# SobeyMIL/MVOC

Measured on AMD Instinct MI355X. Metric: UNet3D denoising steps/sec, 16x512^2 frames, inversion+compose, higher is better.
Workload: dtype f16

## Files before the change

mvoc_amd/csrc/attention.hip:

```cpp
#include <stdlib.h>

#include "common.h"

namespace {

typedef __fp16 fp16x4_t __attribute__((__vector_size__(4 * sizeof(__fp16))));
template <int D> struct FlashPitch { static constexpr int K = 2 * D + 16, V = D == 64 ? 192 : 320; };

struct AttnArgs {
  const half_t *q, *k, *v;
  half_t* out;
  long q_bs, q_ts, k_bs, k_ts, v_bs, v_ts, o_bs, o_ts;
  int nbatch, heads, tq, tk, kv_bdiv, causal;
  float scale_log2;
  long v2_off, o2_off;
  int qblocks;
};

__device__ __forceinline__ int vt_slot_group(int key) {
  return ((((key >> 5) * 2 + ((key >> 4) & 1)) * 2) + ((key >> 2) & 1));
}
__device__ __forceinline__ int vt_slot_elem(int key) { return ((key >> 3) & 1) * 4 + (key & 3); }

constexpr float FLASH_THR = 8.0f;

typedef float f32x2 __attribute__((ext_vector_type(2)));
__device__ __forceinline__ float flash_xhalf_max(float x) {
  const unsigned u = __builtin_bit_cast(unsigned, x);
  const auto sw = __builtin_amdgcn_permlane32_swap(u, u, false, false);
  return fmaxf(__builtin_bit_cast(float, (unsigned)sw[0]), __builtin_bit_cast(float, (unsigned)sw[1]));
}

template <int D, int NV>
#ifndef FLASH_MINW
#define FLASH_MINW 4
#endif
__global__ __launch_bounds__(256, (D == 64 && NV == 1) ? FLASH_MINW : 1) void flash_kernel(const AttnArgs p) {
  constexpr int KPITCH = FlashPitch<D>::K, VPITCH = FlashPitch<D>::V;
  constexpr int ND = D / 16, NT = D / 32, CPK = D / 8, NCH = 64 * CPK / 256;
  __shared__ __attribute__((aligned(16))) char smem[64 * KPITCH + NV * 64 * VPITCH];
  char* Ks = smem;
  char* Vs = smem + 64 * KPITCH;
  const int tid = threadIdx.x, lane = tid & 63;
  const int wave = __builtin_amdgcn_readfirstlane(tid >> 6);
  const int r = lane & 31, h = lane >> 5;
  const unsigned logical = xcd_remap(blockIdx.x, gridDim.x);
  const unsigned qb_ = logical % (unsigned)p.qblocks, hb_ = logical / (unsigned)p.qblocks;
  const int head = (int)(hb_ % (unsigned)p.heads), b = (int)(hb_ / (unsigned)p.heads);
  const int q0 = (int)qb_ * 128 + wave * 32;

  const half_t* qp = p.q + (long)b * p.q_bs + head * D;
  const int qrow = min(q0 + r, p.tq - 1);
  half8_t qf[ND];
#pragma unroll
  for (int s = 0; s < ND; ++s) qf[s] = *reinterpret_cast<const half8_t*>(qp + (long)qrow * p.q_ts + 16 * s + 8 * h);

  const char* kb = reinterpret_cast<const char*>(p.k + (long)(b / p.kv_bdiv) * p.k_bs + head * D);
  const char* vb = reinterpret_cast<const char*>(p.v + (long)(b / p.kv_bdiv) * p.v_bs + head * D);
  const unsigned k_rb = (unsigned)p.k_ts * 2u, v_rb = (unsigned)p.v_ts * 2u;
  unsigned koff[NCH], voff[NCH];
#pragma unroll
  for (int i = 0; i < NCH; ++i) {
    const int c = tid + i * 256;
    koff[i] = (unsigned)(c / CPK) * k_rb + (unsigned)(c % CPK) * 16u;
    voff[i] = (unsigned)(c / CPK) * v_rb + (unsigned)(c % CPK) * 16u;
  }

  f32x16 ot[NV][NT];
#pragma unroll
  for (int v = 0; v < NV; ++v)
#pragma unroll
    for (int dt = 0; dt < NT; ++dt)
#pragma unroll
      for (int e = 0; e < 16; ++e) ot[v][dt][e] = 0.f;
  float mrun = -INFINITY, lrun = 0.f;

  const int ntiles = (p.tk + 63) / 64;
  half8_t kreg[NCH], vreg[NV][NCH];
  auto gload = [&](int kt) {
    const char* kt_ = kb + (size_t)kt * 64u * k_rb;
    const char* vt_ = vb + (size_t)kt * 64u * v_rb;
    const bool ragged = __builtin_amdgcn_readfirstlane(kt * 64 + 64 > p.tk);
#pragma unroll
    for (int i = 0; i < NCH; ++i) {
      unsigned ko = koff[i], vo = voff[i];
      if (ragged) {
        const int c = tid + i * 256;
        const unsigned row = (unsigned)min(c / CPK, p.tk - 1 - kt * 64);
        ko = row * k_rb + (unsigned)(c % CPK) * 16u;
        vo = row * v_rb + (unsigned)(c % CPK) * 16u;
      }
      kreg[i] = *reinterpret_cast<const half8_t*>(kt_ + ko);
#pragma unroll
      for (int v = 0; v < NV; ++v) vreg[v][i] = *reinterpret_cast<const half8_t*>(vt_ + (size_t)v * (size_t)p.v2_off * 2u + vo);
    }
  };
  gload(0);
  for (int kt = 0; kt < ntiles; ++kt) {
    __syncthreads();
#pragma unroll
    for (int i = 0; i < NCH; ++i) {
      const int c = tid + i * 256;
      const int key = c / CPK, dc = c % CPK;
      *reinterpret_cast<half8_t*>(Ks + key * KPITCH + dc * 16) = kreg[i];
#pragma unroll
      for (int v = 0; v < NV; ++v)
        *reinterpret_cast<half8_t*>(Vs + v * 64 * VPITCH + key * VPITCH + dc * 16) = vreg[v][i];
    }
    __syncthreads();
    if (kt + 1 < ntiles) gload(kt + 1);

    f32x16 st[2];
#pragma unroll
    for (int t = 0; t < 2; ++t) {
#pragma unroll
      for (int e = 0; e < 16; ++e) st[t][e] = 0.f;
#pragma unroll
      for (int s = 0; s < ND; ++s) {
        const half8_t kf = *reinterpret_cast<const half8_t*>(Ks + (32 * t + r) * KPITCH + (16 * s + 8 * h) * 2);
        st[t] = __builtin_amdgcn_mfma_f32_32x32x16_f16(kf, qf[s], st[t], 0, 0, 0);
      }
    }
    if (__builtin_amdgcn_readfirstlane((kt == ntiles - 1) && (p.tk & 63))) {
#pragma unroll
      for (int t = 0; t < 2; ++t)
#pragma unroll
        for (int e = 0; e < 16; ++e)
          if (kt * 64 + 32 * t + 8 * (e >> 2) + 4 * h + (e & 3) >= p.tk) st[t][e] = -INFINITY;
    }
    if (p.causal) {
#pragma unroll
      for (int t = 0; t < 2; ++t)
#pragma unroll
        for (int e = 0; e < 16; ++e)
          if (kt * 64 + 32 * t + 8 * (e >> 2) + 4 * h + (e & 3) > q0 + r) st[t][e] = -INFINITY;
    }
    float mx = st[0][0];
#pragma unroll
    for (int t = 0; t < 2; ++t)
#pragma unroll
      for (int e = 0; e < 16; ++e) mx = fmaxf(mx, st[t][e]);
    mx = flash_xhalf_max(mx);
    if (__any((mx - mrun) * p.scale_log2 > FLASH_THR)) {
      const float mnew = fmaxf(mrun, mx);
      const float alpha = __builtin_amdgcn_exp2f((mrun - mnew) * p.scale_log2);
      mrun = mnew;
      lrun *= alpha;
#pragma unroll
      for (int v = 0; v < NV; ++v)
#pragma unroll
        for (int dt = 0; dt < NT; ++dt)
#pragma unroll
          for (int e = 0; e < 16; ++e) ot[v][dt][e] *= alpha;
    }
    const f32x2 sc2 = {p.scale_log2, p.scale_log2}, mc2 = {-mrun * p.scale_log2, -mrun * p.scale_log2};
#pragma unroll
    for (int t = 0; t < 2; ++t)
#pragma unroll
      for (int e = 0; e < 16; e += 2) {
        const f32x2 a = __builtin_elementwise_fma(f32x2{st[t][e], st[t][e + 1]}, sc2, mc2);
        st[t][e] = __builtin_amdgcn_exp2f(a[0]);
        st[t][e + 1] = __builtin_amdgcn_exp2f(a[1]);
      }

#pragma unroll
    for (int t = 0; t < 2; ++t)
#pragma unroll
      for (int s = 0; s < 2; ++s) {
        half8_t pf;
#pragma unroll
        for (int j = 0; j < 8; ++j) pf[j] = (half_t)st[t][8 * s + j];
#pragma unroll
        for (int j = 0; j < 4; ++j) lrun = __builtin_amdgcn_fdot2(half2_t{pf[2 * j], pf[2 * j + 1]}, half2_t{(half_t)1.f, (half_t)1.f}, lrun, false);
        const int krow = 32 * t + 16 * s + 4 * h + ((lane & 15) >> 2);
#pragma unroll
        for (int v = 0; v < NV; ++v)
#pragma unroll
          for (int dt = 0; dt < NT; ++dt) {
            const char* va = Vs + v * 64 * VPITCH + krow * VPITCH + (32 * dt + 16 * ((lane >> 4) & 1) + 4 * (lane & 3)) * 2;
            const fp16x4_t lo = __builtin_amdgcn_ds_read_tr16_b64_v4f16((__attribute__((address_space(3))) fp16x4_t*)va);
            const fp16x4_t hi = __builtin_amdgcn_ds_read_tr16_b64_v4f16((__attribute__((address_space(3))) fp16x4_t*)(va + 8 * VPITCH));
            half8_t vf;
#pragma unroll
            for (int e = 0; e < 4; ++e) {
              vf[e] = (half_t)lo[e];
              vf[4 + e] = (half_t)hi[e];
            }
            ot[v][dt] = __builtin_amdgcn_mfma_f32_32x32x16_f16(vf, pf, ot[v][dt], 0, 0, 0);
          }
      }
  }
  const float ltot = lrun + __shfl_xor(lrun, 32);
  const float inv = 1.0f / ltot;
  int lane_e = tid;
  asm volatile("" : "+v"(lane_e));
  const int r_e = lane_e & 31, h_e = (lane_e >> 5) & 1;
  if (q0 + r_e < p.tq) {
#pragma unroll
    for (int v = 0; v < NV; ++v) {
      half_t* op = p.out + v * p.o2_off + (long)b * p.o_bs + (long)(q0 + r_e) * p.o_ts + head * D;
#pragma unroll
      for (int dt = 0; dt < NT; ++dt)
#pragma unroll
        for (int q = 0; q < 4; ++q) {
          half4_t o;
#pragma unroll
          for (int e = 0; e < 4; ++e) o[e] = (half_t)(ot[v][dt][q * 4 + e] * inv);
          *reinterpret_cast<half4_t*>(op + 32 * dt + 8 * q + 4 * h_e) = o;
        }
    }
  }
}

#define F3_BAR()                         \
  do {                                   \
    __builtin_amdgcn_sched_barrier(0);   \
    __builtin_amdgcn_s_barrier();        \
    __builtin_amdgcn_sched_barrier(0);   \
  } while (0)
#define F3_FENCE() __builtin_amdgcn_sched_barrier(0)
#define F3_GRP(V, T)                                   \
  do {                                                 \
    __builtin_amdgcn_sched_group_barrier(0x008, 1, 0); \
    __builtin_amdgcn_sched_group_barrier(0x002, V, 0); \
    __builtin_amdgcn_sched_group_barrier(0x400, T, 0); \
  } while (0)
#define F3_RD(R) __builtin_amdgcn_sched_group_barrier(0x100, R, 0)
#ifdef MVOC_F3_STAMPS
__device__ unsigned long long f3_dbg[8];
#define F3_STAMP(i)                                                                      \
  do {                                                                                   \
    unsigned long long t_;                                                               \
    asm volatile("s_memtime %0\n\ts_waitcnt lgkmcnt(0)" : "=s"(t_)::"memory");          \
    if (blockIdx.x == 0 && tid == 0) { f3_acc[i] += t_ - f3_last; }                      \
    f3_last = t_;                                                                        \
  } while (0)
#else
#define F3_STAMP(i)
#endif
typedef unsigned u32x4 __attribute__((ext_vector_type(4)));
__device__ __forceinline__ void f3_dma(const u32x4 rsrc, unsigned voff, unsigned lds) {
  unsigned keep;
  asm volatile("s_mov_b32 %0, m0\n\ts_mov_b32 m0, %2\n\ts_nop 0\n\tbuffer_load_dwordx4 %1, %3, 0 offen lds\n\ts_mov_b32 m0, %0"
               : "=&s"(keep) : "v"(voff), "s"(lds), "s"(rsrc) : "memory");
}
__device__ __forceinline__ u32x4 f3_rsrc(const void* base, unsigned bytes) {
  const unsigned long long a = (unsigned long long)base;
  u32x4 r;
  r[0] = __builtin_amdgcn_readfirstlane((unsigned)a);
  r[1] = __builtin_amdgcn_readfirstlane((unsigned)(a >> 32));
  r[2] = __builtin_amdgcn_readfirstlane(bytes);
  r[3] = 0x00020000u;
  return r;
}
template <int N>
__device__ __forceinline__ void f3_wait_vm() {
  asm volatile("s_waitcnt vmcnt(%0)" ::"n"(N) : "memory");
}
#ifndef F3_W1
#define F3_W1 3
#endif
template <int NV>
__global__ __launch_bounds__(256, NV == 1 ? F3_W1 : 2) void flash3_kernel(const AttnArgs p) {
  constexpr int D = 64, NS = (NV == 1 && F3_W1 == 2) ? 4 : 3, TILE = 8192 * (1 + NV), PCS = 2 + 2 * NV;
  __shared__ __attribute__((aligned(1024))) char smem[NS * TILE];
#ifdef MVOC_F3_STAMPS
  unsigned long long f3_acc[6] = {0, 0, 0, 0, 0, 0}, f3_last = 0, f3_t0, f3_r0;
#endif
  const int tid = threadIdx.x, lane = tid & 63;
  const int wave = __builtin_amdgcn_readfirstlane(tid >> 6);
  const int r = lane & 31, h = lane >> 5;
#ifdef MVOC_F3_STAMPS
  asm volatile("s_memtime %0\n\ts_memrealtime %1\n\ts_waitcnt lgkmcnt(0)" : "=s"(f3_t0), "=s"(f3_r0)::"memory");
  f3_last = f3_t0;
#endif
  const unsigned logical = xcd_remap(blockIdx.x, gridDim.x);
  const unsigned qb_ = logical % (unsigned)p.qblocks, hb_ = logical / (unsigned)p.qblocks;
  const int head = (int)(hb_ % (unsigned)p.heads), b = (int)(hb_ / (unsigned)p.heads);
  const int q0 = (int)qb_ * 128 + wave * 32;
  const int nt = (p.tk + 63) >> 6;

  const unsigned k_rb = (unsigned)p.k_ts * 2u, v_rb = (unsigned)p.v_ts * 2u;
  const half_t* kb = p.k + (long)(b / p.kv_bdiv) * p.k_bs + head * D;
  const half_t* vb = p.v + (long)(b / p.kv_bdiv) * p.v_bs + head * D;
  const u32x4 rs_k = f3_rsrc(kb, (unsigned)(p.tk - 1) * k_rb + 128u);
  const u32x4 rs_v0 = f3_rsrc(vb, (unsigned)(p.tk - 1) * v_rb + 128u);
  const u32x4 rs_v1 = f3_rsrc(vb + p.v2_off, (unsigned)(p.tk - 1) * v_rb + 128u);
  unsigned ksrc[2], vsrc[2];
#pragma unroll
  for (int j = 0; j < 2; ++j) {
    const int key_l = 16 * wave + 8 * j + (lane >> 3), pc = lane & 7;
    ksrc[j] = (unsigned)key_l * k_rb + (unsigned)((pc ^ ((key_l >> 1) & 7)) * 16);
    vsrc[j] = (unsigned)key_l * v_rb + (unsigned)((pc ^ (((key_l >> 1) & 1) << 2)) * 16);
  }
  const unsigned ktile = 64u * k_rb, vtile = 64u * v_rb;
  const unsigned lds0 = (unsigned)(size_t)(__attribute__((address_space(3))) char*)smem;
  auto issue = [&](int tile, int so) {
    const unsigned base = lds0 + (unsigned)so + (unsigned)wave * 2048u;
#pragma unroll
    for (int j = 0; j < 2; ++j) f3_dma(rs_k, ksrc[j] + (unsigned)tile * ktile, base + j * 1024);
#pragma unroll
    for (int v = 0; v < NV; ++v)
#pragma unroll
      for (int j = 0; j < 2; ++j) f3_dma(v ? rs_v1 : rs_v0, vsrc[j] + (unsigned)tile * vtile, base + 8192 * (1 + v) + j * 1024);
  };
  const half_t* qp = p.q + (long)b * p.q_bs + head * D;
  const int qrow = min(q0 + r, p.tq - 1);
  half8_t qf[4];
#pragma unroll
  for (int s = 0; s < 4; ++s) qf[s] = *reinterpret_cast<const half8_t*>(qp + (long)qrow * p.q_ts + 16 * s + 8 * h);
  asm volatile("s_nop 4" ::: "memory");
  F3_FENCE();
#pragma unroll
  for (int t = 0; t < NS - 1; ++t) issue(t, t * TILE);
  F3_FENCE();

  f32x16 ot[NV][2];
#pragma unroll
  for (int v = 0; v < NV; ++v)
#pragma unroll
    for (int dt = 0; dt < 2; ++dt)
#pragma unroll
      for (int e = 0; e < 16; ++e) ot[v][dt][e] = 0.f;
  float mrun = -INFINITY, lrun = 0.f;
  f32x16 sa[2], sb[2];
  f32x16 zero16;
#pragma unroll
  for (int e = 0; e < 16; ++e) zero16[e] = 0.f;

  int kfo[4];
#pragma unroll
  for (int s = 0; s < 4; ++s) kfo[s] = r * 128 + (((2 * s + h) ^ ((r >> 1) & 7)) * 16);
  const int vq = (lane & 15) >> 2;
  int vfo[2];
#pragma unroll
  for (int dt = 0; dt < 2; ++dt) vfo[dt] = 8192 + (4 * h + vq) * 128 + (((32 * ((lane >> 4) & 1) + 8 * (lane & 3))) | ((dt ^ ((vq >> 1) & 1)) << 6));

  f3_wait_vm<(NS - 2) * PCS>();
  F3_BAR();
#pragma unroll
  for (int t = 0; t < 2; ++t) {
    sa[t] = zero16;
#pragma unroll
    for (int s = 0; s < 4; ++s) {
      const half8_t kf = *reinterpret_cast<const half8_t*>(smem + kfo[s] + 4096 * t);
      sa[t] = __builtin_amdgcn_mfma_f32_32x32x16_f16(kf, qf[s], sa[t], 0, 0, 0);
    }
  }
  int o_v = 0, o_k = TILE, o_w = (NS - 1) * TILE;

  auto body = [&](f32x16(&cur)[2], f32x16(&nxt)[2], const int t) {
    F3_STAMP(4);
    f3_wait_vm<(NS - 3) * PCS>();
    F3_BAR();
    F3_STAMP(0);
    issue(t + NS - 1, o_w);
    F3_FENCE();
    F3_STAMP(1);
    const char* Kn = smem + o_k;
    const char* Vc = smem + o_v;
    if (__builtin_amdgcn_readfirstlane((t == nt - 1) && (p.tk & 63))) {
#pragma unroll
      for (int tt = 0; tt < 2; ++tt)
#pragma unroll
        for (int e = 0; e < 16; ++e)
          if (t * 64 + 32 * tt + 8 * (e >> 2) + 4 * h + (e & 3) >= p.tk) cur[tt][e] = -INFINITY;
    }
    F3_FENCE();
    half8_t kf[2][4];
#pragma unroll
    for (int s = 0; s < 2; ++s)
#pragma unroll
      for (int tt = 0; tt < 2; ++tt) kf[tt][s] = *reinterpret_cast<const half8_t*>(Kn + kfo[s] + 4096 * tt);
    half8_t pf[2];
    half8_t vf[3][NV][2];
    auto vread = [&](const int f) {
#pragma unroll
      for (int v = 0; v < NV; ++v)
#pragma unroll
        for (int dt = 0; dt < 2; ++dt) {
          const char* va = Vc + 8192 * v + vfo[dt] + (32 * (f >> 1) + 16 * (f & 1)) * 128;
          const fp16x4_t lo = __builtin_amdgcn_ds_read_tr16_b64_v4f16((__attribute__((address_space(3))) fp16x4_t*)va);
          const fp16x4_t hi = __builtin_amdgcn_ds_read_tr16_b64_v4f16((__attribute__((address_space(3))) fp16x4_t*)(va + 8 * 128));
#pragma unroll
          for (int e = 0; e < 4; ++e) {
            vf[f % 3][v][dt][e] = (half_t)lo[e];
            vf[f % 3][v][dt][4 + e] = (half_t)hi[e];
          }
        }
    };
    vread(0);
    F3_FENCE();
    auto smma = [&](const int i) {
      const int tt = i & 1, s_ = i >> 1;
      nxt[tt] = __builtin_amdgcn_mfma_f32_32x32x16_f16(kf[tt][s_], qf[s_], s_ == 0 ? zero16 : nxt[tt], 0, 0, 0);
    };
    auto pvmma = [&](const int f, const int dt) {
#pragma unroll
      for (int v = 0; v < NV; ++v) ot[v][dt] = __builtin_amdgcn_mfma_f32_32x32x16_f16(vf[f % 3][v][dt], pf[f & 1], ot[v][dt], 0, 0, 0);
    };
    float mx = fmaxf(cur[0][0], cur[0][1]);
#pragma unroll
    for (int tt = 0; tt < 2; ++tt)
#pragma unroll
      for (int e = tt ? 0 : 2; e < 16; e += 2) mx = __builtin_fmaxf(__builtin_fmaxf(mx, cur[tt][e]), cur[tt][e + 1]);
    smma(0); smma(1); smma(2);
    if constexpr (NV == 2) smma(3);
    mx = flash_xhalf_max(mx);
    if constexpr (NV == 1) { F3_GRP(6, 0); F3_GRP(6, 0); F3_GRP(6, 0); }
    else { F3_GRP(4, 0); F3_GRP(5, 0); F3_GRP(4, 0); F3_GRP(5, 0); }
    F3_STAMP(2);
    if (__any((mx - mrun) * p.scale_log2 > FLASH_THR)) {
      const float mnew = fmaxf(mrun, mx);
      const float alpha = __builtin_amdgcn_exp2f((mrun - mnew) * p.scale_log2);
      mrun = mnew;
      lrun *= alpha;
#pragma unroll
      for (int v = 0; v < NV; ++v)
#pragma unroll
        for (int dt = 0; dt < 2; ++dt)
#pragma unroll
          for (int e = 0; e < 16; ++e) ot[v][dt][e] *= alpha;
    }
    F3_FENCE();
    const f32x2 sc2 = {p.scale_log2, p.scale_log2}, mc2 = {-mrun * p.scale_log2, -mrun * p.scale_log2};
#pragma unroll
    for (int s = 2; s < 4; ++s)
#pragma unroll
      for (int tt = 0; tt < 2; ++tt) kf[tt][s] = *reinterpret_cast<const half8_t*>(Kn + kfo[s] + 4096 * tt);
#pragma unroll
    for (int f = 0; f < 4; ++f) {
      const int tt = f >> 1, s_ = f & 1;
      if (f < 3) vread(f + 1);
      half8_t& pn = pf[f & 1];
      float x[8];
#pragma unroll
      for (int j = 0; j < 8; j += 2) {
        const f32x2 a = __builtin_elementwise_fma(f32x2{cur[tt][8 * s_ + j], cur[tt][8 * s_ + j + 1]}, sc2, mc2);
        x[j] = __builtin_amdgcn_exp2f(a[0]);
        x[j + 1] = __builtin_amdgcn_exp2f(a[1]);
      }
#pragma unroll
      for (int j = 0; j < 8; ++j) pn[j] = (half_t)x[j];
#pragma unroll
      for (int j = 0; j < 4; ++j) lrun = __builtin_amdgcn_fdot2(half2_t{pn[2 * j], pn[2 * j + 1]}, half2_t{(half_t)1.f, (half_t)1.f}, lrun, false);
      if (f == 0) {
        smma(NV == 1 ? 3 : 4); smma(NV == 1 ? 4 : 5);
        if constexpr (NV == 2) { smma(6); smma(7); } else smma(5);
      } else {
        pvmma(f - 1, 0); pvmma(f - 1, 1);
        if constexpr (NV == 1) { if (f < 3) smma(5 + f); }
      }
    }
    pvmma(3, 0);
    pvmma(3, 1);
    if constexpr (NV == 1) {
      F3_RD(8); F3_GRP(5, 3); F3_GRP(5, 2); F3_GRP(5, 3);
      F3_RD(4); F3_GRP(5, 2); F3_GRP(5, 3); F3_GRP(5, 2);
      F3_RD(4); F3_GRP(5, 3); F3_GRP(5, 2); F3_GRP(5, 3);
      F3_GRP(5, 2); F3_GRP(5, 3); F3_GRP(5, 2); F3_GRP(5, 2);
    } else {
      F3_RD(12); F3_GRP(3, 2); F3_GRP(3, 2); F3_GRP(3, 2); F3_GRP(3, 2);
      F3_RD(8); F3_GRP(3, 2); F3_GRP(3, 2); F3_GRP(3, 2); F3_GRP(3, 2);
      F3_RD(8); F3_GRP(3, 2); F3_GRP(3, 2); F3_GRP(3, 2); F3_GRP(3, 2);
      F3_GRP(3, 2); F3_GRP(3, 2); F3_GRP(3, 2); F3_GRP(3, 2);
      F3_GRP(3, 0); F3_GRP(3, 0); F3_GRP(3, 0); F3_GRP(3, 0);
    }
    F3_FENCE();
    F3_STAMP(3);
    const int o_ = o_v; o_v = o_k;
    o_k = o_k + TILE == NS * TILE ? 0 : o_k + TILE;
    o_w = o_;
  };
#pragma unroll 1
  for (int t = 0;; t += 2) {
    body(sa, sb, t);
    if (t + 1 >= nt) break;
    body(sb, sa, t + 1);
    if (t + 2 >= nt) break;
  }
  f3_wait_vm<0>();
#ifdef MVOC_F3_STAMPS
  if (blockIdx.x == 0 && tid == 0) {
    unsigned long long t1_, r1_;
    asm volatile("s_memtime %0\n\ts_memrealtime %1\n\ts_waitcnt lgkmcnt(0)" : "=s"(t1_), "=s"(r1_)::"memory");
    for (int i = 0; i < 5; ++i) f3_dbg[i] = f3_acc[i];
    f3_dbg[5] = t1_ - f3_t0;
    f3_dbg[7] = r1_ - f3_r0;
    f3_dbg[6] = (unsigned long long)nt;
  }
#endif

  const float ltot = lrun + __shfl_xor(lrun, 32);
  const float inv = 1.0f / ltot;
  if (q0 + r < p.tq) {
#pragma unroll
    for (int v = 0; v < NV; ++v) {
      half_t* op = p.out + v * p.o2_off + (long)b * p.o_bs + (long)(q0 + r) * p.o_ts + head * D;
#pragma unroll
      for (int dt = 0; dt < 2; ++dt)
#pragma unroll
        for (int q = 0; q < 4; ++q) {
          half4_t o;
#pragma unroll
          for (int e = 0; e < 4; ++e) o[e] = (half_t)(ot[v][dt][q * 4 + e] * inv);
          *reinterpret_cast<half4_t*>(op + 32 * dt + 8 * q + 4 * h) = o;
        }
    }
  }
}
#undef F3_BAR
#undef F3_FENCE
#undef F3_GRP
#undef F3_RD
#undef F3_STAMP

struct TAttnArgs {
  const half_t *q, *k, *v;
  half_t* out;
  long q_bs, q_ps, q_ts, k_bs, k_ps, k_ts, v_bs, v_ps, v_ts, o_bs, o_ps, o_ts;
  int nsample, hw, heads, frames;
  int logf, logp, pgroups;
  long ntask;
  float scale_log2;
};

constexpr int TVPITCH = 64;

__global__ __launch_bounds__(256) void tattn_kernel(const TAttnArgs p) {
  __shared__ __attribute__((aligned(16))) char smem[4 * 64 * TVPITCH];
  const int tid = threadIdx.x, lane = tid & 63, wave = tid >> 6;
  const int r = lane & 31, h = lane >> 5;
  char* Vs = smem + wave * 64 * TVPITCH;
  const int F = p.frames, logf = p.logf, P = 1 << p.logp;
  const long task = (long)blockIdx.x * 4 + wave;
  const bool active = task < p.ntask;
  const long tk = active ? task : p.ntask - 1;
  const int head = (int)(tk % p.heads);
  const long bp = tk / p.heads;
  const long smp = bp / p.pgroups, px0 = (bp % p.pgroups) << p.logp;
  const half8_t zero8 = {0, 0, 0, 0, 0, 0, 0, 0};
  auto row_px = [&](int row) { return (long)(P > 1 ? row >> logf : 0); };
  auto row_fr = [&](int row) { return P > 1 ? row & (F - 1) : row; };
  auto row_ok = [&](int row) { return (P > 1 || row < F) && px0 + row_px(row) < p.hw; };

  const half_t* qb = p.q + smp * p.q_bs + px0 * p.q_ps + head * 64;
  const half_t* kb = p.k + smp * p.k_bs + px0 * p.k_ps + head * 64;
  const half_t* vb = p.v + smp * p.v_bs + px0 * p.v_ps + head * 64;

#pragma unroll
  for (int i = 0; i < 4; ++i) {
    const int c = lane + 64 * i;
    const int key = c >> 3, dc = c & 7;
    half8_t vr = zero8;
    if (row_ok(key)) vr = *reinterpret_cast<const half8_t*>(vb + row_px(key) * p.v_ps + (long)row_fr(key) * p.v_ts + dc * 8);
    const int g = (((key >> 4) & 1) * 2) + ((key >> 2) & 1), j = vt_slot_elem(key);
#pragma unroll
    for (int e = 0; e < 8; ++e) {
      const int d = dc * 8 + e;
      *reinterpret_cast<half_t*>(Vs + d * TVPITCH + ((g ^ ((d >> 3) & 3)) * 16) + j * 2) = vr[e];
    }
  }
  f32x16 st;
#pragma unroll
  for (int e = 0; e < 16; ++e) st[e] = 0.f;
  const bool rok = row_ok(r);
  const long koff = row_px(r) * p.k_ps + (long)row_fr(r) * p.k_ts, qoff = row_px(r) * p.q_ps + (long)row_fr(r) * p.q_ts;
#pragma unroll
  for (int s = 0; s < 4; ++s) {
    half8_t kf = zero8, qf = zero8;
    if (rok) {
      kf = *reinterpret_cast<const half8_t*>(kb + koff + 16 * s + 8 * h);
      qf = *reinterpret_cast<const half8_t*>(qb + qoff + 16 * s + 8 * h);
    }
    st = __builtin_amdgcn_mfma_f32_32x32x16_f16(kf, qf, st, 0, 0, 0);
  }
  float mx = -INFINITY;
#pragma unroll
  for (int e = 0; e < 16; ++e) {
    const int key = 8 * (e >> 2) + 4 * h + (e & 3);
    const bool ok = P > 1 ? (key >> logf) == (r >> logf) : key < F;
    const float sv = ok ? st[e] * p.scale_log2 : -INFINITY;
    st[e] = sv;
    mx = fmaxf(mx, sv);
  }
  mx = fmaxf(mx, __shfl_xor(mx, 32));
  float ps = 0.f;
#pragma unroll
  for (int e = 0; e < 16; ++e) {
    const float pv = __builtin_amdgcn_exp2f(st[e] - mx);
    st[e] = pv;
    ps += pv;
  }
  ps += __shfl_xor(ps, 32);
  const float inv = 1.0f / ps;

  __syncthreads();
  f32x16 ot[2];
#pragma unroll
  for (int dt = 0; dt < 2; ++dt)
#pragma unroll
    for (int e = 0; e < 16; ++e) ot[dt][e] = 0.f;
#pragma unroll
  for (int s = 0; s < 2; ++s) {
    half8_t pf;
#pragma unroll
    for (int j = 0; j < 8; ++j) pf[j] = (half_t)st[8 * s + j];
    const int g = s * 2 + h;
#pragma unroll
    for (int dt = 0; dt < 2; ++dt) {
      const int d = 32 * dt + r;
      const half8_t vf = *reinterpret_cast<const half8_t*>(Vs + d * TVPITCH + ((g ^ ((d >> 3) & 3)) * 16));
      ot[dt] = __builtin_amdgcn_mfma_f32_32x32x16_f16(vf, pf, ot[dt], 0, 0, 0);
    }
  }
  if (active && rok) {
    half_t* op = p.out + smp * p.o_bs + (px0 + row_px(r)) * p.o_ps + (long)row_fr(r) * p.o_ts + head * 64;
#pragma unroll
    for (int dt = 0; dt < 2; ++dt)
#pragma unroll
      for (int q = 0; q < 4; ++q) {
        half4_t o;
#pragma unroll
        for (int e = 0; e < 4; ++e) o[e] = (half_t)(ot[dt][q * 4 + e] * inv);
        *reinterpret_cast<half4_t*>(op + 32 * dt + 8 * q + 4 * h) = o;
      }
  }
}

}

static const int g_f3_env = getenv("MVOC_FLASH3") ? atoi(getenv("MVOC_FLASH3")) : -1;

extern "C" int mvoc_flash_attn_f16(const mvoc_attn_desc* d, void* stream) {
  MVOC_REQUIRE(d && d->q && d->k && d->v && d->out, -1, "flash_attn: null operand");
  MVOC_REQUIRE(d->nbatch > 0 && d->heads > 0 && d->tq > 0 && d->tk > 0, -1, "flash_attn: empty problem");
  MVOC_REQUIRE(d->nbatch <= 65535 && d->heads <= 65535, -2, "flash_attn: grid too large");
  MVOC_REQUIRE(d->q_ts % 8 == 0 && d->k_ts % 8 == 0 && d->v_ts % 8 == 0 && d->o_ts % 4 == 0, -2,
               "flash_attn: row strides must keep 16-byte alignment");
  AttnArgs a;
  a.q = (const half_t*)d->q; a.k = (const half_t*)d->k; a.v = (const half_t*)d->v; a.out = (half_t*)d->out;
  a.q_bs = d->q_bs; a.q_ts = d->q_ts; a.k_bs = d->k_bs; a.k_ts = d->k_ts; a.v_bs = d->v_bs; a.v_ts = d->v_ts;
  a.o_bs = d->o_bs; a.o_ts = d->o_ts;
  a.nbatch = d->nbatch; a.heads = d->heads; a.tq = d->tq; a.tk = d->tk; a.kv_bdiv = d->kv_bdiv > 0 ? d->kv_bdiv : 1;
  const int hd = d->head_dim > 0 ? d->head_dim : 64;
  MVOC_REQUIRE(hd == 64 || hd == 96, -2, "flash_attn: head_dim (%d) must be 64 or 96", hd);
  MVOC_REQUIRE(!d->causal || d->tq == d->tk, -2, "flash_attn: the causal form is self-attention (tq == tk)");
  a.causal = d->causal;
  a.scale_log2 = (d->scale > 0.f ? d->scale : (hd == 64 ? 0.125f : 1.0f / sqrtf((float)hd))) * 1.4426950408889634f;
  hipStream_t s = (hipStream_t)stream;
  MvocProfScope prof(MVOC_FAM_FLASH, s, (d->v2 ? 2.0 : 1.0) * 4.0 * d->nbatch * d->heads * (double)d->tq * d->tk * hd);
  a.qblocks = (d->tq + 127) / 128;
  const long nblk = (long)a.qblocks * d->heads * d->nbatch;
  MVOC_REQUIRE(nblk < 0x7fffffffL, -2, "flash_attn: grid too large");
  dim3 grid((unsigned)nblk);
  a.v2_off = a.o2_off = 0;
  MVOC_REQUIRE(d->pipelined >= 0 && d->pipelined <= 2, -1, "flash_attn: pipelined must be 0 (by key count), 1 (never) or 2 (wherever it applies)");
  const int f3_mode = d->pipelined ? d->pipelined - 1 : g_f3_env;
  const bool pipelined = hd == 64 && !d->causal && (f3_mode >= 0 ? f3_mode != 0 : d->tk >= 2048);
  if (d->v2) {
    MVOC_REQUIRE(d->out2 && hd == 64, -2, "flash_attn: the paired form needs out2 and head_dim 64");
    a.v2_off = (const half_t*)d->v2 - a.v;
    a.o2_off = (half_t*)d->out2 - a.out;
    MVOC_REQUIRE(a.v2_off % 8 == 0 && a.o2_off % 4 == 0, -2, "flash_attn: v2 / out2 must keep 16-byte alignment");
    if (pipelined) hipLaunchKernelGGL((flash3_kernel<2>), grid, dim3(256), 0, s, a);
    else hipLaunchKernelGGL((flash_kernel<64, 2>), grid, dim3(256), 0, s, a);
  } else if (hd == 64) {
    if (pipelined) hipLaunchKernelGGL((flash3_kernel<1>), grid, dim3(256), 0, s, a);
    else hipLaunchKernelGGL((flash_kernel<64, 1>), grid, dim3(256), 0, s, a);
  } else {
    hipLaunchKernelGGL((flash_kernel<96, 1>), grid, dim3(256), 0, s, a);
  }
  return mvoc_check_launch("flash_kernel");
}

#ifdef MVOC_F3_STAMPS
extern "C" int mvoc_f3_stamps_read(unsigned long long* host8) {
  return hipMemcpyFromSymbol(host8, HIP_SYMBOL(f3_dbg), sizeof(unsigned long long) * 8) == hipSuccess ? 0 : -1;
}
#endif

extern "C" int mvoc_temporal_attn_f16(const mvoc_tattn_desc* d, void* stream) {
  MVOC_REQUIRE(d && d->q && d->k && d->v && d->out, -1, "temporal_attn: null operand");
  MVOC_REQUIRE(d->nsample > 0 && d->hw > 0 && d->heads > 0, -1, "temporal_attn: empty problem");
  MVOC_REQUIRE(d->frames >= 1 && d->frames <= 32, -2, "temporal_attn: frames (%d) must be in [1, 32]", d->frames);
  MVOC_REQUIRE(d->q_ts % 8 == 0 && d->k_ts % 8 == 0 && d->v_ts % 8 == 0 && d->o_ts % 4 == 0 && d->q_ps % 8 == 0 &&
                   d->k_ps % 8 == 0 && d->v_ps % 8 == 0 && d->o_ps % 4 == 0,
               -2, "temporal_attn: strides must keep 16-byte alignment");
  TAttnArgs a;
  a.q = (const half_t*)d->q; a.k = (const half_t*)d->k; a.v = (const half_t*)d->v; a.out = (half_t*)d->out;
  a.q_bs = d->q_bs; a.q_ps = d->q_ps; a.q_ts = d->q_ts; a.k_bs = d->k_bs; a.k_ps = d->k_ps; a.k_ts = d->k_ts;
  a.v_bs = d->v_bs; a.v_ps = d->v_ps; a.v_ts = d->v_ts; a.o_bs = d->o_bs; a.o_ps = d->o_ps; a.o_ts = d->o_ts;
  a.nsample = d->nsample; a.hw = d->hw; a.heads = d->heads; a.frames = d->frames;
  a.logf = d->frames == 8 ? 3 : d->frames == 16 ? 4 : 5;
  a.logp = d->frames == 8 ? 2 : d->frames == 16 ? 1 : 0;
  a.pgroups = (d->hw + (1 << a.logp) - 1) >> a.logp;
  a.ntask = (long)d->nsample * a.pgroups * d->heads;
  a.scale_log2 = 0.125f * 1.4426950408889634f;
  const long nblk = (a.ntask + 3) / 4;
  MVOC_REQUIRE(nblk < 0x7fffffffL, -2, "temporal_attn: grid too large");
  hipStream_t s = (hipStream_t)stream;
  MvocProfScope prof(MVOC_FAM_TATTN, s, 4.0 * (double)d->nsample * d->hw * d->heads * d->frames * 64 * 2);
  hipLaunchKernelGGL(tattn_kernel, dim3((unsigned)nblk), dim3(256), 0, s, a);
  return mvoc_check_launch("tattn_kernel");
}
```

Baseline: 24.33.

## Add persistent streaming temporal-attention kernel with register prefetch of next task

Adds a persistent-grid temporal attention kernel in which each wave walks a strided list of tasks. It prefetches the next task's Q/K/V into registers while computing the current one, and stages the output through LDS so global stores are coalesced 16-byte writes. The aim is to hide global load latency and cut block launch overhead for the many small per-pixel attention tasks. It is enabled by default when frames are 8 or 16 and the output is 16-byte aligned; otherwise the old kernel runs. Costs include extra register pressure and a grid capped at 3 blocks per CU, which may limit occupancy.

Result: no change. 24.54, median of 6 (+0.9%).

```diff
diff --git a/mvoc_amd/csrc/attention.hip b/mvoc_amd/csrc/attention.hip
--- a/mvoc_amd/csrc/attention.hip
+++ b/mvoc_amd/csrc/attention.hip
@@ -628,9 +628,161 @@
   }
 }
 
+constexpr int TS_WAVE_LDS = 3 * 4096;
+
+__global__ __launch_bounds__(256) void tattn_kernel_stream(const TAttnArgs p, const int niter) {
+  __shared__ __attribute__((aligned(16))) char smem[4 * TS_WAVE_LDS];
+  const int tid = threadIdx.x, lane = tid & 63;
+  const int wave = __builtin_amdgcn_readfirstlane(tid >> 6);
+  const int r = lane & 31, h = lane >> 5;
+  char* Qs = smem + wave * TS_WAVE_LDS;
+  char* Ks = Qs + 4096;
+  char* Vs = Qs + 8192;
+  const int F = p.frames, logf = p.logf;
+  const unsigned ntask = (unsigned)p.ntask, stride = gridDim.x * 4u;
+  unsigned task = blockIdx.x * 4u + (unsigned)wave;
+  if (task >= ntask) return;
+  const half8_t zero8 = {0, 0, 0, 0, 0, 0, 0, 0};
+
+  const int lr = lane >> 3, lc = lane & 7;
+  const long ql = (long)lr * p.q_ts + lc * 8, kl = (long)lr * p.k_ts + lc * 8, vl = (long)lr * p.v_ts + lc * 8, ol = (long)lr * p.o_ts + lc * 8;
+  auto piece_px = [&](int i) { return (long)((8 * i) >> logf); };
+  auto piece_fr = [&](int i) { return (long)((8 * i) & (F - 1)); };
+  auto qk_at = [&](int row, int chunk) { return row * 128 + ((chunk ^ ((row >> 1) & 7)) * 16); };
+  auto v_at = [&](int row, int chunk) { return row * 128 + ((chunk ^ (((row >> 1) & 1) << 2)) * 16); };
+  auto decode = [&](unsigned t, long& smp, long& px0, int& head) {
+    head = (int)(t % (unsigned)p.heads);
+    const unsigned bp = t / (unsigned)p.heads;
+    smp = (long)(bp / (unsigned)p.pgroups);
+    px0 = (long)(bp % (unsigned)p.pgroups) << p.logp;
+  };
+
+  half8_t qr[4], kr[4], vr[4];
+  auto gload = [&](long smp, long px0, int head) {
+    const half_t* qb = p.q + smp * p.q_bs + px0 * p.q_ps + head * 64;
+    const half_t* kb = p.k + smp * p.k_bs + px0 * p.k_ps + head * 64;
+    const half_t* vb = p.v + smp * p.v_bs + px0 * p.v_ps + head * 64;
+#pragma unroll
+    for (int i = 0; i < 4; ++i) {
+      qr[i] = zero8;
+      kr[i] = zero8;
+      vr[i] = zero8;
+      if (px0 + piece_px(i) < p.hw) {
+        qr[i] = *reinterpret_cast<const half8_t*>(qb + piece_px(i) * p.q_ps + piece_fr(i) * p.q_ts + ql);
+        kr[i] = *reinterpret_cast<const half8_t*>(kb + piece_px(i) * p.k_ps + piece_fr(i) * p.k_ts + kl);
+        vr[i] = *reinterpret_cast<const half8_t*>(vb + piece_px(i) * p.v_ps + piece_fr(i) * p.v_ts + vl);
+      }
+    }
+  };
+
+  long smp, px0;
+  int head;
+  decode(task, smp, px0, head);
+  gload(smp, px0, head);
+#pragma unroll 1
+  for (int it = 0; it < niter; ++it) {
+#pragma unroll
+    for (int i = 0; i < 4; ++i) {
+      const int row = 8 * i + lr;
+      *reinterpret_cast<half8_t*>(Qs + qk_at(row, lc)) = qr[i];
+      *reinterpret_cast<half8_t*>(Ks + qk_at(row, lc)) = kr[i];
+      *reinterpret_cast<half8_t*>(Vs + v_at(row, lc)) = vr[i];
+    }
+    asm volatile("" ::: "memory");
+    const unsigned next = task + stride;
+    const bool more = __builtin_amdgcn_readfirstlane((it + 1 < niter) && (next < ntask));
+    long nsmp = smp, npx0 = px0;
+    int nhead = head;
+    if (more) {
+      decode(next, nsmp, npx0, nhead);
+      gload(nsmp, npx0, nhead);
+    }
+    asm volatile("" ::: "memory");
+
+    f32x16 st;
+#pragma unroll
+    for (int e = 0; e < 16; ++e) st[e] = 0.f;
+#pragma unroll
+    for (int s = 0; s < 4; ++s) {
+      const half8_t kf = *reinterpret_cast<const half8_t*>(Ks + qk_at(r, 2 * s + h));
+      const half8_t qf = *reinterpret_cast<const half8_t*>(Qs + qk_at(r, 2 * s + h));
+      st = __builtin_amdgcn_mfma_f32_32x32x16_f16(kf, qf, st, 0, 0, 0);
+    }
+    float mx = -INFINITY;
+#pragma unroll
+    for (int e = 0; e < 16; ++e) {
+      const int key = 8 * (e >> 2) + 4 * h + (e & 3);
+      const bool ok = (key >> logf) == (r >> logf);
+      const float sv = ok ? st[e] * p.scale_log2 : -INFINITY;
+      st[e] = sv;
+      mx = fmaxf(mx, sv);
+    }
+    mx = fmaxf(mx, __shfl_xor(mx, 32));
+    float ps = 0.f;
+#pragma unroll
+    for (int e = 0; e < 16; ++e) {
+      const float pv = __builtin_amdgcn_exp2f(st[e] - mx);
+      st[e] = pv;
+      ps += pv;
+    }
+    ps += __shfl_xor(ps, 32);
+    const float inv = 1.0f / ps;
+
+    f32x16 ot[2];
+#pragma unroll
+    for (int dt = 0; dt < 2; ++dt)
+#pragma unroll
+      for (int e = 0; e < 16; ++e) ot[dt][e] = 0.f;
+    const int vq = (lane & 15) >> 2;
+#pragma unroll
+    for (int s = 0; s < 2; ++s) {
+      half8_t pf;
+#pragma unroll
+      for (int j = 0; j < 8; ++j) pf[j] = (half_t)st[8 * s + j];
+#pragma unroll
+      for (int dt = 0; dt < 2; ++dt) {
+        const char* va = Vs + (16 * s + 4 * h + vq) * 128 + ((32 * ((lane >> 4) & 1) + 8 * (lane & 3)) | ((dt ^ ((vq >> 1) & 1)) << 6));
+        const fp16x4_t lo = __builtin_amdgcn_ds_read_tr16_b64_v4f16((__attribute__((address_space(3))) fp16x4_t*)va);
+        const fp16x4_t hi = __builtin_amdgcn_ds_read_tr16_b64_v4f16((__attribute__((address_space(3))) fp16x4_t*)(va + 8 * 128));
+        half8_t vf;
+#pragma unroll
+        for (int e = 0; e < 4; ++e) {
+          vf[e] = (half_t)lo[e];
+          vf[4 + e] = (half_t)hi[e];
+        }
+        ot[dt] = __builtin_amdgcn_mfma_f32_32x32x16_f16(vf, pf, ot[dt], 0, 0, 0);
+      }
+    }
+    asm volatile("" ::: "memory");
+#pragma unroll
+    for (int dt = 0; dt < 2; ++dt)
+#pragma unroll
+      for (int q = 0; q < 4; ++q) {
+        half4_t o;
+#pragma unroll
+        for (int e = 0; e < 4; ++e) o[e] = (half_t)(ot[dt][q * 4 + e] * inv);
+        *reinterpret_cast<half4_t*>(Qs + qk_at(r, 4 * dt + q) + 8 * h) = o;
+      }
+    asm volatile("" ::: "memory");
+    half_t* ob = p.out + smp * p.o_bs + px0 * p.o_ps + head * 64;
+#pragma unroll
+    for (int i = 0; i < 4; ++i) {
+      const half8_t o = *reinterpret_cast<const half8_t*>(Qs + qk_at(8 * i + lr, lc));
+      if (px0 + piece_px(i) < p.hw) *reinterpret_cast<half8_t*>(ob + piece_px(i) * p.o_ps + piece_fr(i) * p.o_ts + ol) = o;
+    }
+    asm volatile("" ::: "memory");
+    if (!more) break;
+    task = next;
+    smp = nsmp;
+    px0 = npx0;
+    head = nhead;
+  }
+}
+
 }
 
 static const int g_f3_env = getenv("MVOC_FLASH3") ? atoi(getenv("MVOC_FLASH3")) : -1;
+static const int g_tstream_env = getenv("MVOC_TATTN_STREAM") ? atoi(getenv("MVOC_TATTN_STREAM")) : 1;
 
 extern "C" int mvoc_flash_attn_f16(const mvoc_attn_desc* d, void* stream) {
   MVOC_REQUIRE(d && d->q && d->k && d->v && d->out, -1, "flash_attn: null operand");
@@ -701,6 +853,18 @@
   MVOC_REQUIRE(nblk < 0x7fffffffL, -2, "temporal_attn: grid too large");
   hipStream_t s = (hipStream_t)stream;
   MvocProfScope prof(MVOC_FAM_TATTN, s, 4.0 * (double)d->nsample * d->hw * d->heads * d->frames * 64 * 2);
+  const bool o16 = (uintptr_t)d->out % 16 == 0 && d->o_bs % 8 == 0 && d->o_ps % 8 == 0 && d->o_ts % 8 == 0;
+  if (g_tstream_env != 0 && a.logp > 0 && o16 && a.ntask < 0x7fffffffL) {
+    static const int ncu = [] {
+      int dev = 0, n = 0;
+      if (hipGetDevice(&dev) != hipSuccess || hipDeviceGetAttribute(&n, hipDeviceAttributeMultiprocessorCount, dev) != hipSuccess || n <= 0) n = 256;
+      return n;
+    }();
+    const long grid = nblk < 3L * ncu ? nblk : 3L * ncu;
+    const int niter = (int)((nblk + grid - 1) / grid);
+    hipLaunchKernelGGL(tattn_kernel_stream, dim3((unsigned)grid), dim3(256), 0, s, a, niter);
+    return mvoc_check_launch("tattn_kernel_stream");
+  }
   hipLaunchKernelGGL(tattn_kernel, dim3((unsigned)nblk), dim3(256), 0, s, a);
   return mvoc_check_launch("tattn_kernel");
 }
```
